# marl/l3embedding

Hardware: AMD Instinct MI355X
Metric: AVC training pairs/sec (1s audio + 224x224 frame) (higher is better)
Workload: dtype f32; 1 GPU; full cnn_L3_melspec2 AVC training step (audio+vision+fusion, fwd+bwd+Adam), batch 64 per GPU, global batch 64, fp32, inputs resident in HBM; global_batch=64, parallelism=dp1, fp32_conv=f4x4

## Files before the change

### l3embedding_amd/csrc/bn_fused.hip

```cpp
#include "kernels.h"
#include "device_common.h"

namespace l3 {



__device__ __forceinline__ void store_quad(void* base, int64_t q, f32x4 v, int obf) {
    if (obf) {
        bf16x4 h;
        h[0] = (__bf16)v.x; h[1] = (__bf16)v.y; h[2] = (__bf16)v.z; h[3] = (__bf16)v.w;
        __builtin_nontemporal_store(h, reinterpret_cast<bf16x4*>(base) + q);
    } else {
        __builtin_nontemporal_store(v, reinterpret_cast<f32x4*>(base) + q);
    }
}

template <bool XBF>
__device__ __forceinline__ f32x4 load_quad(const void* base, int64_t q) {
    if constexpr (XBF) {
        const u32x2 r = __builtin_nontemporal_load(reinterpret_cast<const u32x2*>(base) + q);
        return f32x4{__uint_as_float(r.x << 16), __uint_as_float(r.x & 0xffff0000u), __uint_as_float(r.y << 16),
                     __uint_as_float(r.y & 0xffff0000u)};
    } else {
        return __builtin_nontemporal_load(reinterpret_cast<const f32x4*>(base) + q);
// ... 545 lines not shown
    using ReduceFn = void (*)(const void*, const void*, const f32x4*, const f32x4*, const f32x4*, const f32x4*, float*, int64_t,
                              Pool2Geom, float, int);
    static const ReduceFn reduce_fns[8] = {
        bn_bwd_reduce_fast_kernel<false, false, false>, bn_bwd_reduce_fast_kernel<false, false, true>,
        bn_bwd_reduce_fast_kernel<false, true, false>,  bn_bwd_reduce_fast_kernel<false, true, true>,
        bn_bwd_reduce_fast_kernel<true, false, false>,  bn_bwd_reduce_fast_kernel<true, false, true>,
        bn_bwd_reduce_fast_kernel<true, true, false>,   bn_bwd_reduce_fast_kernel<true, true, true>};
    if (ready_part != nullptr) {
        launch_fast_final(BwdFinal{gamma, mean, var, dgamma, dbeta, cA, cB, cC, 1.0 / (double)rows, eps, training}, ready_part,
                          ready_blocks, C, s);
    } else {
        hipLaunchKernelGGL(reduce_fns[variant], dim3(nb_r), dim3(FB), 0, s, xv, dyv, sc4, sh4, reinterpret_cast<const f32x4*>(mean),
                           reinterpret_cast<const f32x4*>(var), part, n4, g, eps, relu);
        launch_fast_final(BwdFinal{gamma, mean, var, dgamma, dbeta, cA, cB, cC, 1.0 / (double)rows, eps, training}, part,
                          nb_r, C, s);
    }
    if (dx == nullptr) return;
    const int64_t work_a = pooled ? (int64_t)N * g.Hc * g.Wc * (C / 4) : n4;
    const int nb_a = fast_blocks(work_a);
    float* part2 = dbias ? part : nullptr;
    using ApplyFn = void (*)(const void*, const void*, const f32x4*, const f32x4*, const f32x4*, const f32x4*, const f32x4*, void*,
                             float*, int64_t, Pool2Geom, int, int);
    static const ApplyFn apply_fns[8] = {
        bn_bwd_apply_fast_kernel<false, false, false>, bn_bwd_apply_fast_kernel<false, false, true>,
        bn_bwd_apply_fast_kernel<false, true, false>,  bn_bwd_apply_fast_kernel<false, true, true>,
        bn_bwd_apply_fast_kernel<true, false, false>,  bn_bwd_apply_fast_kernel<true, false, true>,
        bn_bwd_apply_fast_kernel<true, true, false>,   bn_bwd_apply_fast_kernel<true, true, true>};
    hipLaunchKernelGGL(apply_fns[variant], dim3(nb_a), dim3(FB), 0, s, xv, dyv, sc4, sh4, reinterpret_cast<const f32x4*>(cA),
                       reinterpret_cast<const f32x4*>(cB), reinterpret_cast<const f32x4*>(cC), (void*)dx, part2, n4, g, relu,
                       dx_bf16);
    if (dbias) launch_fast_final(SumFinal{dbias}, part, nb_a, C, s);
}

}
```

### l3embedding_amd/csrc/elementwise.hip

```cpp
#include "kernels.h"

namespace l3 {

static constexpr int RED_BLOCK = 256;
static constexpr int RED_MAX_BLOCKS = 1024;
static constexpr int SMALLC_MAX = 16;

static inline int red_blocks(int64_t rows, int C) {
    int rows_per_pass = (C % 4 == 0 && C >= 4 && C <= 1024) ? (RED_BLOCK / (C / 4) > 0 ? RED_BLOCK / (C / 4) : 1) : RED_BLOCK;
    int64_t b = (rows + (int64_t)rows_per_pass * 16 - 1) / ((int64_t)rows_per_pass * 16);
    if (b < 1) b = 1;
    if (b > RED_MAX_BLOCKS) b = RED_MAX_BLOCKS;
    return (int)b;
}

size_t colreduce_scratch_floats(int64_t rows, int C) {
    const size_t a = (size_t)red_blocks(rows, C) * 2 * (size_t)(C < 4 ? 4 : C) + 64;
    const size_t b = bn_fast_ok(C) ? bn_fast_scratch_floats(C) : 0;
    return a > b ? a : b;
}

template <class F>
__global__ __launch_bounds__(RED_BLOCK) void colreduce_vec_kernel(F f, float* part, int64_t rows, int C) {
    __shared__ float sm[2][RED_BLOCK * 4];
// ... 494 lines not shown
    float best[4];
    int arg[4];
    gp_scan(x + (size_t)n * P * C + cb * 64 + cq * 4, P, C, pg, best, arg);
    gp_merge(sb, sa, pg, cq, best, arg);
    if (threadIdx.x < 64) y[(size_t)n * out_batch_stride + cb * 64 + threadIdx.x] = sb[0][threadIdx.x];
}
__global__ __launch_bounds__(256) void global_maxpool_bwd_kernel(const float* __restrict__ x, const float* __restrict__ dy,
                                                                 float* __restrict__ dx, int P, int C,
                                                                 int64_t out_batch_stride) {
    __shared__ float sb[16][64];
    __shared__ int sa[16][64];
    const int cb = blockIdx.x % (C / 64), n = blockIdx.x / (C / 64);
    const int cq = threadIdx.x & 15, pg = threadIdx.x >> 4;
    float best[4];
    int arg[4];
    const size_t base = (size_t)n * P * C + cb * 64 + cq * 4;
    gp_scan(x + base, P, C, pg, best, arg);
    gp_merge(sb, sa, pg, cq, best, arg);
    const gp4 d = *reinterpret_cast<const gp4*>(dy + (size_t)n * out_batch_stride + cb * 64 + cq * 4);
    int am[4];
#pragma unroll
    for (int e = 0; e < 4; ++e) am[e] = sa[0][cq * 4 + e];
    for (int p = pg; p < P; p += 16) {
        gp4 o;
#pragma unroll
        for (int e = 0; e < 4; ++e) o[e] = p == am[e] ? d[e] : 0.f;
        *reinterpret_cast<gp4*>(dx + base + (size_t)p * C) = o;
    }
}
static bool is_global_pool(const PoolGeom& g) {
    return g.Ho == 1 && g.Wo == 1 && g.padT == 0 && g.padL == 0 && g.ph == g.H && g.pw == g.W && g.C % 64 == 0 &&
           g.out_batch_stride % 4 == 0;
}

void maxpool_fwd(const float* x, float* y, const PoolGeom& g, hipStream_t s) {
    if (is_global_pool(g)) {
        hipLaunchKernelGGL(global_maxpool_fwd_kernel, dim3(g.N * (g.C / 64)), dim3(256), 0, s, x, y, g.H * g.W, g.C,
                           (int64_t)g.out_batch_stride);
        return;
    }
    const int64_t total = (int64_t)g.N * g.Ho * g.Wo * g.C;
    hipLaunchKernelGGL(maxpool_fwd_kernel, dim3(ew_blocks(total)), dim3(256), 0, s, x, y, g);
}
__global__ __launch_bounds__(256) void maxpool_bwd_kernel(const float* x, const float* dy, float* dx, PoolGeom g) {
    const int64_t total = (int64_t)g.N * g.Ho * g.Wo * g.C;
    for (int64_t i = (int64_t)blockIdx.x * 256 + threadIdx.x; i < total; i += (int64_t)gridDim.x * 256) {
        const int c = (int)(i % g.C);
        int64_t r = i / g.C;
        const int wo = (int)(r % g.Wo);
        r /= g.Wo;
        const int ho = (int)(r % g.Ho);
        const int n = (int)(r / g.Ho);
        const int h0 = ho * g.sh - g.padT, w0 = wo * g.sw - g.padL;
        float best = -INFINITY;
        int ba = -1, bb = -1;
        for (int a = 0; a < g.ph; ++a) {
            const int h = h0 + a;
            if ((unsigned)h >= (unsigned)g.H) continue;
            for (int b = 0; b < g.pw; ++b) {
                const int w = w0 + b;
                if ((unsigned)w >= (unsigned)g.W) continue;
                const float v = x[((size_t)(n * g.H + h) * g.W + w) * g.C + c];
                if (ba < 0 || v > best) { best = v; ba = a; bb = b; }
            }
        }
        const float d = dy[(size_t)n * g.out_batch_stride + ((size_t)ho * g.Wo + wo) * g.C + c];
// ... 32 lines not shown
        xa[i] = c == C ? 1.f : (x[r * C + c] - mean[c]) * (1.f / sqrtf(var[c] + eps));
    }
}
void bn_xhat_ones(const float* x, const float* mean, const float* var, float eps, float* xa, int64_t rows, int C,
                  hipStream_t s) {
    hipLaunchKernelGGL(bn_xhat_ones_kernel, dim3(ew_blocks(rows * (C + 1))), dim3(256), 0, s, x, mean, var, eps, xa, rows, C);
}

__global__ __launch_bounds__(256) void first_conv_grads_kernel(const float* __restrict__ gaug, const float* __restrict__ w,
                                                               const float* __restrict__ gamma, const float* __restrict__ beta,
                                                               float* __restrict__ dw, float* __restrict__ dgamma,
                                                               float* __restrict__ dbeta, float* __restrict__ dbias, int taps,
                                                               int C, int Co) {
    __shared__ double red[2][256];
    const int t = threadIdx.x;
    const int C1 = C + 1;
    for (int i = t; i < taps * C * Co; i += 256) {
        const int co = i % Co, ci = (i / Co) % C, tap = i / (Co * C);
        dw[i] = gamma[ci] * gaug[(tap * C1 + ci) * Co + co] + beta[ci] * gaug[(tap * C1 + C) * Co + co];
    }
    if (dbias != nullptr)
        for (int co = t; co < Co; co += 256) dbias[co] = gaug[((taps / 2) * C1 + C) * Co + co];
    for (int ci = 0; ci < C; ++ci) {
        double sg = 0.0, sb = 0.0;
        for (int i = t; i < taps * Co; i += 256) {
            const int co = i % Co, tap = i / Co;
            const double wv = (double)w[(tap * C + ci) * Co + co];
            sg += wv * (double)gaug[(tap * C1 + ci) * Co + co];
            sb += wv * (double)gaug[(tap * C1 + C) * Co + co];
        }
        red[0][t] = sg;
        red[1][t] = sb;
        __syncthreads();
        if (t == 0) {
            double a = 0.0, b = 0.0;
            for (int k = 0; k < 256; ++k) {
                a += red[0][k];
                b += red[1][k];
            }
            dgamma[ci] = (float)a;
            dbeta[ci] = (float)b;
        }
        __syncthreads();
    }
}
void first_conv_grads(const float* gaug, const float* w, const float* gamma, const float* beta, float* dw, float* dgamma,
                      float* dbeta, float* dbias, int taps, int C, int Co, hipStream_t s) {
    hipLaunchKernelGGL(first_conv_grads_kernel, dim3(1), dim3(256), 0, s, gaug, w, gamma, beta, dw, dgamma, dbeta, dbias, taps,
                       C, Co);
}

__global__ __launch_bounds__(256) void preprocess_video_kernel(const uint8_t* u8, float* out, int64_t n) {
    for (int64_t i = (int64_t)blockIdx.x * 256 + threadIdx.x; i < n; i += (int64_t)gridDim.x * 256) {
        const float f = (float)((double)u8[i] / 255.0);
        out[i] = 2.f * f - 1.f;
    }
}
__global__ __launch_bounds__(256) void preprocess_audio_kernel(const int16_t* pcm, float* out, int64_t n) {
    for (int64_t i = (int64_t)blockIdx.x * 256 + threadIdx.x; i < n; i += (int64_t)gridDim.x * 256)
        out[i] = (float)pcm[i] / 32768.f;
}
__global__ void labels_onehot_kernel(const int32_t* lab, float* out, int64_t n) {
    for (int64_t i = (int64_t)blockIdx.x * blockDim.x + threadIdx.x; i < n; i += (int64_t)gridDim.x * blockDim.x)
        out[i] = (float)lab[i];
}
void preprocess_video(const uint8_t* u8, float* out, int64_t n, hipStream_t s) {
    hipLaunchKernelGGL(preprocess_video_kernel, dim3(ew_blocks(n)), dim3(256), 0, s, u8, out, n);
}
void preprocess_audio(const int16_t* pcm, float* out, int64_t n, hipStream_t s) {
    hipLaunchKernelGGL(preprocess_audio_kernel, dim3(ew_blocks(n)), dim3(256), 0, s, pcm, out, n);
}
void labels_onehot(const int32_t* lab, float* out, int64_t n, hipStream_t s) {
    hipLaunchKernelGGL(labels_onehot_kernel, dim3(ew_blocks(n)), dim3(256), 0, s, lab, out, n);
}
// ... 231 lines not shown
```

### l3embedding_amd/csrc/engine.hip

```cpp
#include <hip/hip_runtime.h>
#include "knobs.h"

#include <cmath>
#include <cstdio>
#include <cstdlib>
#include <cstring>
#include <map>
#include <string>
#include <vector>

#include "../../include/l3hip.h"
#include "comm.h"
#include "kernels.h"

namespace {

using namespace l3;

static thread_local std::string g_create_error;

constexpr float BN_EPS = 1e-3f;
constexpr float BN_MOMENTUM = 0.99f;
constexpr float L2_WEIGHT = 1e-5f;
constexpr float ADAM_B1 = 0.9f, ADAM_B2 = 0.999f, ADAM_EPS = 1e-8f;
// ... 16 lines not shown

struct Param {
    std::string name;
    int ndim = 0;
    int64_t shape[4] = {1, 1, 1, 1};
    bool trainable = false;
    int kind = 0;
    int64_t numel = 0;
    int bucket = 0;
    float* d = nullptr;
    float* g = nullptr;
};

enum ConvFwd { CF_BF16_STORED, CF_BF16_CAST, CF_FIRST, CF_FP32 };
enum ConvWgrad { WG_AUG, WG_AUG_DEFERRED, WG_BF16_STORED, WG_BF16_CAST, WG_FP32 };
enum ConvDgrad { DG_NONE, DG_SMALL, DG_BF16_STORED, DG_BF16_CAST, DG_WINO, DG_FLIPPED };
struct ConvPlan {
    ConvFwd fwd = CF_FP32;
    bool wino_filter = false;
    int stat_mode = 0;
    ConvWgrad wgrad = WG_FP32;
    bool colsum = false;
    ConvDgrad dgrad = DG_NONE;
    int bwd_bn = -1;
    double fwd_executed = -1.0, fwd_bytes = 0.0, wg_executed = -1.0, wg_bytes = 0.0, dg_executed = -1.0, dg_bytes = 0.0;
};
enum BnStats { BS_PARTIALS, BS_FAST, BS_PLAIN, BS_MOVING };
enum BnBwd { BB_BY_FIRST_CONV, BB_FAST_POOLED, BB_FAST, BB_FAST_DEFERRED, BB_PLAIN };
struct BnPlan {
    BnStats stats = BS_MOVING;
    int stat_blocks = 0;
    BnBwd bwd = BB_PLAIN;
    int bwd_blocks = 0;
    double fwd_bytes = 0.0, bwd_bytes = 0.0;
};

struct Op {
    OpKind kind;
    std::string name;
    int in = 0, out = 0;
    int block = 0, bucket = 0;
    int kh = 0, kw = 0, cout = 0;
    bool same = false;
    ConvGeom geom{};
    ConvGeom dgeom{};
    int p_kernel = -1, p_bias = -1;
    float* wflip = nullptr;
    float *wino_uf = nullptr, *wino_ud = nullptr;
    int in_bn = -1;
    bool fused_first = false;
    bool defer_apply = false;
    int bn_defer = -1;
    float *xaug = nullptr, *gaug = nullptr;
    ConvGeom ageom{};
    int bn_follow = -1;
    bool need_dx = true;
    int dy_to_bn = -1;
    float* xwin = nullptr;
    int p_gamma = -1, p_beta = -1, p_mmean = -1, p_mvar = -1;
    bool fused_relu = false;
    bool prerelu = false;
    int fuse_pool = -1;
    int bias_param = -1;
    bool fused_into_bn = false;
    bool bias_by_bn = false;
    float *mean = nullptr, *var = nullptr, *scale = nullptr, *shift = nullptr;
    float *biased_mean = nullptr, *biased_var = nullptr;
    PoolGeom pg{};
    ConvPlan cp{};
    BnPlan bp{};
};

struct Tower {
    std::string prefix;
    std::vector<Tensor> t;
    std::vector<Op> ops;
    int nblocks = 0;
    int emb_conv_op = -1;
    bool training = false;
};

struct FrontendDef {
    int n_dft, n_hop, same, n_mels, sqrt_out, db, loglambda;
    const char* layer_name;
};

struct ProfRec {
    int family;
    hipEvent_t a, b;
    double flops;
    double executed;
// ... 889 lines not shown
                    const size_t sf = (size_t)conv_wino_stat_blocks_max(op.geom) * 2 * op.geom.Cout;
                    if (sf > stat_max) stat_max = sf;
                    const size_t sb = (size_t)conv_bf16_stat_blocks(op.geom) * 2 * op.geom.Cout;
                    if (e->cfg.dtype == L3_DTYPE_BF16 && sb > stat_max) stat_max = sb;
                    const size_t s1 = (size_t)conv_first_stat_blocks(op.geom) * 2 * op.geom.Cout;
                    if (s1 > stat_max) stat_max = s1;
                    const size_t sd = op.dy_to_bn >= 0 ? (size_t)conv_wino_stat_blocks_max(op.dgeom) * 2 * op.dgeom.Cout : 0;
                    if (sd > stat_max) stat_max = sd;
                    const size_t sdb = op.dy_to_bn >= 0 && e->cfg.dtype == L3_DTYPE_BF16
                                           ? (size_t)conv_bf16_stat_blocks(op.dgeom) * 2 * op.dgeom.Cout : 0;
                    if (sdb > stat_max) stat_max = sdb;
                }
                if (op.need_dx && conv_wino_floats(op.dgeom) &&
                    (rc = dev_alloc_t(e, &op.wino_ud, conv_wino_floats(op.dgeom))))
                    return rc;
                const size_t w = conv_wgrad_scratch_floats(op.geom);
                if (w > wg_max) wg_max = w;
                if (op.in_bn >= 0) {
                    if ((rc = dev_alloc_t(e, &op.xaug, (size_t)x.rows() * op.ageom.Cin))) return rc;
                    if ((rc = dev_alloc_t(e, &op.gaug, (size_t)op.kh * op.kw * op.ageom.Cin * op.cout))) return rc;
                    const size_t wa = conv_wgrad_scratch_floats(op.ageom);
                    if (wa > wg_max) wg_max = wa;
                }
                const size_t r = colreduce_scratch_floats(y.rows(), y.C);
                if (r > red_max) red_max = r;
            } else if (op.kind == OP_BN) {
                const int C = x.C;
                for (float** p : {&op.mean, &op.var, &op.scale, &op.shift, &op.biased_mean, &op.biased_var}) {
                    if ((rc = dev_alloc_t(e, p, (size_t)(C + 3) / 4 * 4))) return rc;
                    HIPCHK(e, hipMemset(*p, 0, (size_t)(C + 3) / 4 * 4 * 4));
                }
                const size_t r = colreduce_scratch_floats(x.rows(), C);
                if (r > red_max) red_max = r;
            }
        }
    }
    if (e->vis.ops.back().kind != OP_POOL || e->aud.ops.back().kind != OP_POOL) {
        e->err = "tower must end in a pooling layer";
        return L3_EINVAL;
    }
    if ((rc = dev_alloc_t(e, &e->red_scratch, red_max))) return rc;
    if ((rc = dev_alloc_t(e, &e->wg_scratch, wg_max))) return rc;
    if ((rc = dev_alloc_t(e, &e->sq_scratch, 2048))) return rc;
    if (stat_max && (rc = dev_alloc_t(e, &e->stat_scratch, stat_max))) return rc;
    {
        bool any_w4 = false;
        for (Tower* tw : {&e->vis, &e->aud})
            for (auto& op : tw->ops)
                if (op.kind == OP_CONV && (op.wino_uf || op.wino_ud)) any_w4 = true;
        if (any_w4 && e->cfg.dtype != L3_DTYPE_BF16 && (rc = dev_alloc_t(e, &e->w4_tail, conv_wino4_tail_scratch_bytes() / sizeof(float)))) return rc;
    }
    if (e->side) {
        if ((rc = dev_alloc_t(e, &e->red_scratch2, red_max))) return rc;
        if ((rc = dev_alloc_t(e, &e->wg_scratch2, wg_max))) return rc;
        if (stat_max && (rc = dev_alloc_t(e, &e->stat_scratch2, stat_max))) return rc;
    }
    return L3_OK;
}

int run_frontend(l3_engine* e) {
    int rc = rebuild_consts(e);
    if (rc) return rc;
    const FrontendCfg& f = e->fcfg;
    const int B = e->B;
    const int M = B * f.n_frames;
    if (f.factored) {
// ... 96 lines not shown
            p.wg_bytes = (double)x.rows() * op.ageom.Cin * 4.0 + (fb ? act_bytes(tw.t[fb->in]) + grad_bytes(tw.t[fb->out]) : grad_bytes(y));
            continue;
        }
        const bool wbf = bf16 && conv_wgrad_bf16_ok(op.geom);
        p.wgrad = !wbf ? WG_FP32 : x.d_bf16 && y.g_bf16 ? WG_BF16_STORED : WG_BF16_CAST;
        p.wg_executed = conv_wgrad_executed_flops(op.geom, wbf);
        p.wg_bytes = act_bytes(x) + grad_bytes(y) + wbytes;
        p.colsum = !op.bias_by_bn;
        if (!op.need_dx) continue;
        const bool dbf = bf16 && conv_bf16_ok(op.dgeom);
        p.dgrad = conv_dgrad_small_ok(op.geom) ? DG_SMALL
                  : dbf                        ? (y.g_bf16 ? DG_BF16_STORED : DG_BF16_CAST)
                  : op.wino_ud                 ? DG_WINO : DG_FLIPPED;
        p.dg_executed = op.wino_ud && !dbf ? conv_wino_executed_flops(op.dgeom) : -1.0;
        p.dg_bytes = grad_bytes(y) + grad_bytes(x) + wbytes;
        Op* bn = training && op.dy_to_bn >= 0 && e->stat_max > 0 ? &tw.ops[op.dy_to_bn] : nullptr;
        if (bn != nullptr && bn->fuse_pool >= 0 && (bn->xwin == nullptr || x.batch_stride != (int64_t)x.H * x.W * x.C)) bn = nullptr;
        if (bn == nullptr) continue;
        const bool bx = tw.t[bn->in].d_bf16;
        int blocks = -1;
        if (p.dgrad == DG_BF16_STORED && x.g_bf16 && bx && conv_bf16_halo_ok(op.dgeom)) blocks = conv_bf16_stat_blocks(op.dgeom);
        if (p.dgrad == DG_WINO && !x.g_bf16 && !bx && conv_wino_ok(op.dgeom)) blocks = conv_wino_stat_blocks(op.dgeom);
        if (blocks < 0) continue;
        if (!fits(op, blocks, op.dgeom.Cout)) return L3_ESTATE;
        p.bwd_bn = op.dy_to_bn;
        bn->bp.bwd_blocks = blocks;
    }
    for (auto& op : tw.ops) {
        if (op.kind != OP_BN) continue;
        const Tensor &x = tw.t[op.in], &y = tw.t[op.out];
        const Tensor& out = op.fuse_pool >= 0 ? tw.t[tw.ops[op.fuse_pool].out] : y;
        BnPlan& p = op.bp;
        p.stats = !training ? BS_MOVING : p.stat_blocks > 0 ? BS_PARTIALS : op.prerelu || x.d_bf16 ? BS_FAST : BS_PLAIN;
        p.bwd = training && op.fused_first ? BB_BY_FIRST_CONV : !bn_fast_ok(x.C) ? BB_PLAIN : op.fuse_pool >= 0 ? BB_FAST_POOLED
                : defers(op) ? BB_FAST_DEFERRED : BB_FAST;
        p.fwd_bytes = (!training ? 0.0 : p.stat_blocks > 0 ? (double)p.stat_blocks * 2 * x.C * 4 : act_bytes(x)) + act_bytes(x) + act_bytes(out);
        if (p.bwd == BB_BY_FIRST_CONV) p.fwd_bytes += act_bytes(x) + (double)x.rows() * (&op + 1)->ageom.Cin * 4.0;
        if (op.fuse_pool >= 0 && training && op.xwin != nullptr) p.fwd_bytes += (double)out.numel() * (x.d_bf16 ? 2.0 : 4.0);
        p.bwd_bytes = p.bwd == BB_PLAIN ? 2.0 * (act_bytes(x) + grad_bytes(y)) + grad_bytes(x)
                                        : (p.bwd_blocks > 0 ? (double)p.bwd_blocks * 2 * x.C * 4 : act_bytes(x) + grad_bytes(out)) +
                                              (p.bwd == BB_FAST_DEFERRED ? 0.0 : act_bytes(x) + grad_bytes(out) + grad_bytes(x));
    }
    return L3_OK;
}

void tower_forward(l3_engine* e, Tower& tw) {
    const bool training = tw.training;
    for (auto& op : tw.ops) {
        Tensor& x = tw.t[op.in];
        Tensor& y = tw.t[op.out];
        switch (op.kind) {
            case OP_CONV: {
                const ConvPlan& p = op.cp;
                const float *w = e->params[op.p_kernel].d, *bias = e->params[op.p_bias].d;
                float* part = p.stat_mode ? e->stat_scratch : nullptr;
                ProfScope ps(e, F_CONV_FWD, conv_flops(op.geom), op.name.c_str(), p.fwd_executed);
                ps.bytes(p.fwd_bytes);
                if (p.wino_filter) conv_wino_transform_weights(w, op.wino_uf, op.geom, false, e->stream);
                switch (p.fwd) {
                    case CF_BF16_STORED:
                        conv_weights_bf16(w, op.wflip, op.kh, op.kw, x.C, op.cout, true, e->stream);
                        conv_bf16_fwd(x.d, op.wflip, bias, y.d, op.geom, e->stream, true, part, p.stat_mode, y.d_bf16);
                        break;
                    case CF_BF16_CAST:
                        conv_flip_weights(w, op.wflip, op.kh, op.kw, x.C, op.cout, e->stream);
                        conv_bf16_fwd(x.d, op.wflip, bias, y.d, op.geom, e->stream);
                        break;
                    case CF_FIRST:
                        conv_first_fwd(x.d, w, bias, y.d, op.geom, e->stream, part, p.stat_mode, y.d_bf16);
                        break;
                    case CF_FP32:
                        conv_fwd(x.d, w, bias, y.d, op.geom, e->stream, p.wino_filter ? op.wino_uf : nullptr, part, p.stat_mode);
                        break;
                }
                break;
            }
            case OP_BN: {
                const BnPlan& p = op.bp;
                ProfScope ps(e, F_ELEMWISE, 0.0);
                ps.bytes(p.fwd_bytes);
                const float* gamma = e->params[op.p_gamma].d;
                const float* beta = e->params[op.p_beta].d;
                switch (p.stats) {
                    case BS_PARTIALS:
                        bn_stats_from_partials(e->stat_scratch, p.stat_blocks, e->params[op.bias_param].d, gamma, beta, op.mean, op.var,
                                               op.scale, op.shift, x.rows(), x.C, BN_EPS, op.prerelu ? 1 : 0, e->stream);
                        break;
                    case BS_FAST:
                        bn_stats_fast(x.d, gamma, beta, op.mean, op.var, op.scale, op.shift, e->red_scratch, x.rows(), x.C, BN_EPS,
                                      op.prerelu ? 1 : 0, e->stream, x.d_bf16 ? 1 : 0);
                        break;
                    case BS_PLAIN:
                        bn_stats(x.d, gamma, beta, op.mean, op.var, op.scale, op.shift, e->red_scratch, x.rows(), x.C, BN_EPS, e->stream);
                        break;
                    case BS_MOVING:
                        bn_scale_shift(gamma, beta, e->params[op.p_mmean].d, e->params[op.p_mvar].d, op.scale, op.shift, x.C, BN_EPS,
                                       e->stream);
                        break;
                }
                if (p.bwd == BB_BY_FIRST_CONV) bn_xhat_ones(x.d, op.mean, op.var, BN_EPS, (&op + 1)->xaug, x.rows(), x.C, e->stream);
                if (op.fuse_pool >= 0) {
                    Tensor& pl = tw.t[tw.ops[op.fuse_pool].out];
                    bn_relu_pool2_fwd(x.d, op.scale, op.shift, pl.d, x.N, x.H, x.W, x.C, pl.H, pl.W, pl.batch_stride,
                                      op.prerelu ? 2 : (op.fused_relu ? 1 : 0), e->stream, pl.d_bf16 ? 1 : 0, x.d_bf16 ? 1 : 0,
                                      training ? (void*)op.xwin : nullptr);
                } else if (y.d_bf16 || x.d_bf16) {
                    bn_apply_fast(x.d, op.scale, op.shift, y.d, x.rows(), x.C, op.fused_relu ? 1 : 0, e->stream, y.d_bf16 ? 1 : 0,
                                  x.d_bf16 ? 1 : 0);
                } else {
                    bn_apply(x.d, op.scale, op.shift, y.d, x.rows(), x.C, op.fused_relu ? 1 : 0, e->stream);
                }
                break;
            }
            case OP_RELU: {
                if (op.fused_into_bn) break;
                ProfScope ps(e, F_ELEMWISE, 0.0);
                ps.bytes(act_bytes(x) + act_bytes(y));
                relu_fwd(x.d, y.d, x.numel(), e->stream);
                break;
            }
            case OP_POOL: {
                if (op.fused_into_bn) break;
                ProfScope ps(e, F_ELEMWISE, 0.0);
                ps.bytes(act_bytes(x) + act_bytes(y));
                maxpool_fwd(x.d, y.d, op.pg, e->stream);
                break;
            }
            default: break;
        }
    }
}

BnBwdFuse bn_bwd_fuse(const Tower& tw, const Op& bn) {
    return BnBwdFuse{bn.fuse_pool >= 0 ? bn.xwin : tw.t[bn.in].d, bn.scale, bn.shift, bn.mean, bn.var, BN_EPS, bn.fused_relu ? 1 : 0};
}

void tower_backward_block(l3_engine* e, Tower& tw, int block) {
    const bool training = tw.training;
    for (int oi = (int)tw.ops.size() - 1; oi >= 0; --oi) {
        Op& op = tw.ops[oi];
        if (op.block != block) continue;
        Tensor& x = tw.t[op.in];
        Tensor& y = tw.t[op.out];
        switch (op.kind) {
            case OP_POOL: {
                if (op.fused_into_bn) break;
                ProfScope ps(e, F_ELEMWISE, 0.0);
                ps.bytes(act_bytes(x) + grad_bytes(y) + grad_bytes(x));
                maxpool_bwd(x.d, y.g, x.g, op.pg, e->stream);
                break;
            }
            case OP_RELU: {
                if (op.fused_into_bn) break;
                ProfScope ps(e, F_ELEMWISE, 0.0);
                ps.bytes(act_bytes(y) + grad_bytes(y) + grad_bytes(x));
                relu_bwd(y.d, y.g, x.g, x.numel(), e->stream);
                break;
            }
            case OP_BN: {
                const BnPlan& p = op.bp;
                if (p.bwd == BB_BY_FIRST_CONV) break;
                ProfScope ps(e, F_ELEMWISE, 0.0);
                ps.bytes(p.bwd_bytes);
                const float* mean = training ? op.mean : e->params[op.p_mmean].d;
                const float* var = training ? op.var : e->params[op.p_mvar].d;
                const float* gamma = e->params[op.p_gamma].d;
                float *dgamma = e->params[op.p_gamma].g, *dbeta = e->params[op.p_beta].g;
                if (p.bwd == BB_PLAIN) {
                    bn_bwd(x.d, y.d, y.g, gamma, mean, var, x.g, dgamma, dbeta, e->red_scratch, x.rows(), x.C, BN_EPS, op.fused_relu ? 1 : 0,
                           training ? 1 : 0, e->stream);
                    break;
                }
                const bool pooled = p.bwd == BB_FAST_POOLED, defer = p.bwd == BB_FAST_DEFERRED;
                const Tensor& dy = pooled ? tw.t[tw.ops[op.fuse_pool].out] : y;
                bn_bwd_fast(x.d, op.scale, op.shift, mean, var, gamma, dy.g, pooled ? 1 : 0, x.N, x.H, x.W, x.C, dy.H, dy.W,
                            pooled ? dy.batch_stride : (int64_t)x.H * x.W * x.C, defer ? nullptr : x.g, dgamma, dbeta,
                            defer ? nullptr : op.bias_param >= 0 ? e->params[op.bias_param].g : nullptr, e->red_scratch, BN_EPS,
                            pooled ? (op.prerelu ? 2 : 1) : (op.fused_relu ? 1 : 0), training ? 1 : 0, e->stream, x.g_bf16 ? 1 : 0,
                            x.d_bf16 ? 1 : 0, dy.g_bf16 ? 1 : 0, p.bwd_blocks > 0 ? e->stat_scratch : nullptr, p.bwd_blocks);
                break;
            }
            case OP_CONV: {
                const ConvPlan& p = op.cp;
                const float* w = e->params[op.p_kernel].d;
                if (p.wgrad == WG_AUG || p.wgrad == WG_AUG_DEFERRED) {
                    ProfScope ps(e, F_CONV_WGRAD, conv_flops(op.geom), op.name.c_str());
                    ps.bytes(p.wg_bytes);
                    const Op& bn = tw.ops[op.in_bn];
                    if (p.wgrad == WG_AUG_DEFERRED) {
                        const Op& fb = tw.ops[op.bn_defer];
                        const Tensor &bi = tw.t[fb.in], &bo = tw.t[fb.out];
                        const float* co = bn_bwd_fast_coeffs(e->red_scratch, op.cout);
                        const FirstWgFuse f{bi.d, bo.g, fb.scale, fb.shift, co, co + op.cout, co + 2 * op.cout, fb.fused_relu ? 1 : 0,
                                            bi.d_bf16 ? 1 : 0};
                        conv_wgrad(op.xaug, nullptr, op.gaug, e->wg_scratch, op.ageom, e->stream, false, false, &f);
                    } else {
                        conv_wgrad(op.xaug, y.g, op.gaug, e->wg_scratch, op.ageom, e->stream);
                    }
                    first_conv_grads(op.gaug, w, e->params[bn.p_gamma].d, e->params[bn.p_beta].d, e->params[op.p_kernel].g,
                                     e->params[bn.p_gamma].g, e->params[bn.p_beta].g,
// ... 1309 lines not shown
int l3_activation_numel(l3_engine* e, const char* name, int64_t* numel) {
    if (!e || !name || !numel) return L3_EINVAL;
    const std::string nm(name);
    if (nm == "h0") { *numel = (int64_t)e->B * (e->nv + e->na); return L3_OK; }
    if (nm == "h1") { *numel = (int64_t)e->B * e->head; return L3_OK; }
    if (nm == "logits" || nm == "probs") { *numel = (int64_t)e->B * 2; return L3_OK; }
    Tensor* t = nullptr;
    if (!find_tower_tensor(e, nm, &t)) {
        e->err = "unknown activation: " + nm;
        return L3_EINVAL;
    }
    *numel = t->numel();
    return L3_OK;
}

int l3_get_activation(l3_engine* e, const char* name, float* dst, int64_t numel) {
    int64_t n = 0;
    int rc = l3_activation_numel(e, name, &n);
    if (rc) return rc;
    if (n != numel) {
        e->err = "activation size mismatch";
        return L3_EINVAL;
    }
    HIPCHK(e, hipSetDevice(e->cfg.device));
    HIPCHK(e, l3::stream_wait(e->stream));
    const std::string nm(name);
    const float* src = nullptr;
    if (nm == "h0") src = e->h0;
    else if (nm == "h1") src = e->h1;
    else if (nm == "logits") src = e->logits;
    else if (nm == "probs") src = e->probs;
    else {
        Tensor* t = nullptr;
        find_tower_tensor(e, nm, &t);
        if (t->alias || t->d == nullptr) {
            e->err = "activation is not materialised (aliased into h0 or fused away)";
            return L3_EINVAL;
        }
        src = t->d;
        if (t->d_bf16) {
            std::vector<uint16_t> h((size_t)numel);
            HIPCHK(e, hipMemcpy(h.data(), src, (size_t)numel * 2, hipMemcpyDeviceToHost));
            l3::widen_bf16(dst, h.data(), (size_t)numel);
            return L3_OK;
        }
    }
    HIPCHK(e, hipMemcpy(dst, src, (size_t)numel * 4, hipMemcpyDeviceToHost));
    return L3_OK;
}

int l3_sync(l3_engine* e) {
    if (!e) return L3_EINVAL;
    HIPCHK(e, hipSetDevice(e->cfg.device));
    HIPCHK(e, l3::stream_wait(e->stream));
    if (e->side) HIPCHK(e, l3::stream_wait(e->side));
    prof_collect(e);
    return L3_OK;
}

int l3_set_tower_overlap(l3_engine* e, int on) {
    if (!e) return L3_EINVAL;
    HIPCHK(e, l3::stream_wait(e->stream));
    if (e->side) HIPCHK(e, l3::stream_wait(e->side));
    e->overlap = on != 0;
    return L3_OK;
}

int l3_profile_enable(l3_engine* e, int on) {
// ... 44 lines not shown
```

### l3embedding_amd/csrc/kernels.h

```cpp
#pragma once
#include <hip/hip_runtime.h>
#include <stdint.h>

#include <string>
#include <vector>

#include "host_common.h"

namespace l3 {

struct ConvGeom {
    int N, H, W, Cin;
    int Ho, Wo, Cout;
    int KH, KW, padT, padL;
    int f2x2 = 0;
    int solo = 0;
    int dynamic = 0;
    float* tail_scratch = nullptr;
    size_t tail_scratch_bytes = 0;
};
size_t conv_wino4_tail_scratch_bytes();

struct BnBwdFuse {
    const float* x;
// ... 79 lines not shown
                      int zero_debias, int step, hipStream_t s);
int* persistent_work_counters(hipStream_t s);

struct BnMovingEntry {
    float* moving;
    float* biased;
    const float* batch;
    int C;
    int off;
};
void bn_moving_update_all(const BnMovingEntry* tab_dev, int entries, int max_c, float momentum, int zero_debias, int64_t step,
                          hipStream_t s, const float* gathered = nullptr, int replicas = 1, int64_t stride = 0);
void bn_moving_pack(const BnMovingEntry* tab_dev, int entries, int max_c, float* packed, hipStream_t s);

bool bn_fast_ok(int C);
size_t bn_fast_scratch_floats(int C);
void bn_stats_fast(const float* x, const float* gamma, const float* beta, float* mean, float* var, float* scale,
                   float* shift, float* scratch, int64_t rows, int C, float eps, int prerelu, hipStream_t s, int x_bf16 = 0);
void bn_stats_from_partials(const float* part, int nblk, const float* pivot, const float* gamma, const float* beta,
                            float* mean, float* var, float* scale, float* shift, int64_t rows, int C, float eps,
                            int prerelu, hipStream_t s);
void bn_apply_fast(const float* x, const float* scale, const float* shift, float* y, int64_t rows, int C, int relu,
                   hipStream_t s, int out_bf16 = 0, int x_bf16 = 0);
void bn_relu_pool2_fwd(const float* x, const float* scale, const float* shift, float* p, int N, int H, int W, int C,
                       int Ho, int Wo, int64_t out_batch_stride, int mode, hipStream_t s, int out_bf16 = 0, int x_bf16 = 0,
                       void* xwin = nullptr);
void bn_bwd_fast(const float* x, const float* scale, const float* shift, const float* mean, const float* var,
                 const float* gamma, const float* dy, int pooled, int N, int H, int W, int C, int Ho, int Wo,
                 int64_t dy_batch_stride, float* dx, float* dgamma, float* dbeta, float* dbias, float* scratch,
                 float eps, int relu, int training, hipStream_t s, int dx_bf16 = 0, int x_bf16 = 0, int dy_bf16 = 0,
                 const float* ready_part = nullptr, int ready_blocks = 0);
const float* bn_bwd_fast_coeffs(const float* scratch, int C);

void relu_fwd(const float* x, float* y, int64_t n, hipStream_t s);
void relu_bwd(const float* y, const float* dy, float* dx, int64_t n, hipStream_t s);

struct PoolGeom {
    int N, H, W, C, Ho, Wo, ph, pw, sh, sw, padT, padL;
    int64_t out_batch_stride;
};
void maxpool_fwd(const float* x, float* y, const PoolGeom& g, hipStream_t s);
void maxpool_bwd(const float* x, const float* dy, float* dx, const PoolGeom& g, hipStream_t s);

void preprocess_video(const uint8_t* u8, float* out, int64_t n, hipStream_t s);
void preprocess_audio(const int16_t* pcm, float* out, int64_t n, hipStream_t s);
void labels_onehot(const int32_t* lab, float* out, int64_t n, hipStream_t s);

struct AugmentParams {
    int32_t start_x, start_y, flip, sat_first;
    float saturation, brightness;
};
constexpr int AUG_CROP = 224;
void augment_video(const uint8_t* u8, int N, int H, int W, const AugmentParams* params, uint8_t* out_u8, float* out_f32,
                   hipStream_t s);
void augment_audio(const int16_t* pcm, int N, int T, const double* u, int16_t* out_i16, float* out_f32, double* gains,
                   hipStream_t s);

struct FrontendCfg {
    int n_dft, n_hop, pad_left, n_frames, n_freq, n_mels;
    int sqrt_out;
    int db;
    int loglambda;
    int ncols_pad;
    int folded, ke, ko, nc;
    int factored, N1, N2;
};
void dft_pack_frames(const float* audio, const float* win, float* a1, int B, int T, const FrontendCfg& c, hipStream_t s);
void dft_twiddle(const float* y, const float* tw, float* a2, float* nyq, int frames, const FrontendCfg& c, hipStream_t s);
void frame_audio_folded(const float* audio, float* fe, float* fo, int B, int T, const FrontendCfg& c, hipStream_t s);
void frame_audio(const float* audio, float* frames, int B, int T, const FrontendCfg& c, hipStream_t s);
void dft_fused(const float* audio, const float* win, const float* b1, const float* b2, const float* tw, const float* melw,
               const int* mel_start, const int* mel_len, const int* mel_off, float* out, int B, int T, const FrontendCfg& c,
               hipStream_t s);
// ... 71 lines not shown
```

Before: 2017 pairs/s.

## Fuse tower-final BN+ReLU with global max-pool in forward and backward

When a tower's last BN (with fused ReLU) feeds a global max-pool, the forward now computes BN+ReLU on the fly and reduces straight to the pooled output plus argmax indices, so the full post-BN activation is never written. The backward rebuilds the sparse pooled gradient from the stored indices inside the BN backward reduce and apply kernels, skipping the separate maxpool backward pass and its dense gradient tensor. It also swaps the serial 256-element double reduction in first_conv_grads for a tree reduction. In exchange it adds scratch and index buffers, and the BN output tensor is no longer readable for debugging.

```diff
diff --git a/l3embedding_amd/csrc/bn_fused.hip b/l3embedding_amd/csrc/bn_fused.hip
--- a/l3embedding_amd/csrc/bn_fused.hip
+++ b/l3embedding_amd/csrc/bn_fused.hip
@@ -601,4 +601,172 @@
     if (dbias) launch_fast_final(SumFinal{dbias}, part, nb_a, C, s);
 }
 
-}
+constexpr int GP_MAX_SLICES = 32;
+static inline int gpool_slices(int P) {
+    const int s = (P + 15) / 16;
+    return s < 1 ? 1 : s > GP_MAX_SLICES ? GP_MAX_SLICES : s;
+}
+size_t bn_relu_gpool_scratch_floats(int N, int C) { return (size_t)N * GP_MAX_SLICES * C * 2; }
+
+__global__ __launch_bounds__(FB) void bn_relu_gpool_fwd_kernel(const f32x4* __restrict__ x, const f32x4* scale, const f32x4* shift,
+                                                              float* __restrict__ pval, int* __restrict__ pidx, int P, int C4,
+                                                              int slices, int chunk) {
+    __shared__ f32x4 sb[FB];
+    __shared__ int sa[FB][4];
+    const int t = threadIdx.x, c4 = t % C4, pg = t / C4, G = FB / C4;
+    const int n = blockIdx.x / slices, sl = blockIdx.x - n * slices;
+    const int p0 = sl * chunk, p1 = min(P, p0 + chunk);
+    const f32x4 sc = scale[c4], sh = shift[c4];
+    const f32x4* xb = x + (size_t)n * P * C4 + c4;
+    f32x4 best = {-INFINITY, -INFINITY, -INFINITY, -INFINITY};
+    int arg[4] = {0x7fffffff, 0x7fffffff, 0x7fffffff, 0x7fffffff};
+#pragma unroll 4
+    for (int p = p0 + pg; p < p1; p += G) {
+        const f32x4 v = relu4(bn_pre(xb[(size_t)p * C4], sc, sh));
+#pragma unroll
+        for (int e = 0; e < 4; ++e)
+            if (v[e] > best[e] || arg[e] == 0x7fffffff) {
+                best[e] = v[e];
+                arg[e] = p;
+            }
+    }
+    sb[t] = best;
+#pragma unroll
+    for (int e = 0; e < 4; ++e) sa[t][e] = arg[e];
+    __syncthreads();
+    if (pg == 0) {
+        for (int k = 1; k < G; ++k) {
+            const f32x4 vb = sb[k * C4 + c4];
+#pragma unroll
+            for (int e = 0; e < 4; ++e) {
+                const int va = sa[k * C4 + c4][e];
+                if (vb[e] > best[e] || (vb[e] == best[e] && va < arg[e])) {
+                    best[e] = vb[e];
+                    arg[e] = va;
+                }
+            }
+        }
+        const size_t o = ((size_t)blockIdx.x * C4 + c4) * 4;
+        *reinterpret_cast<f32x4*>(pval + o) = best;
+#pragma unroll
+        for (int e = 0; e < 4; ++e) pidx[o + e] = arg[e];
+    }
+}
+__global__ __launch_bounds__(256) void bn_relu_gpool_merge_kernel(const float* __restrict__ pval, const int* __restrict__ pidx,
+                                                                  float* __restrict__ p, int* __restrict__ win, int N, int C,
+                                                                  int slices, int64_t out_batch_stride) {
+    const int i = blockIdx.x * 256 + threadIdx.x;
+    if (i >= N * C) return;
+    const int n = i / C, c = i - n * C;
+    float vs[GP_MAX_SLICES];
+    int as[GP_MAX_SLICES];
+#pragma unroll
+    for (int sl = 0; sl < GP_MAX_SLICES; ++sl) {
+        const size_t o = ((size_t)n * slices + (sl < slices ? sl : 0)) * C + c;
+        vs[sl] = pval[o];
+        as[sl] = sl < slices ? pidx[o] : 0x7fffffff;
+    }
+    float b = -INFINITY;
+    int a = 0x7fffffff;
+#pragma unroll
+    for (int sl = 0; sl < GP_MAX_SLICES; ++sl)
+        if (as[sl] != 0x7fffffff && (vs[sl] > b || a == 0x7fffffff)) {
+            b = vs[sl];
+            a = as[sl];
+        }
+    p[(size_t)n * out_batch_stride + c] = b;
+    win[i] = a;
+}
+void bn_relu_gpool_fwd(const float* x, const float* scale, const float* shift, float* p, int* win, float* scratch, int N, int P, int C,
+                       int64_t out_batch_stride, hipStream_t s) {
+    const int slices = gpool_slices(P), chunk = (P + slices - 1) / slices;
+    float* pval = scratch;
+    int* pidx = reinterpret_cast<int*>(scratch + (size_t)N * slices * C);
+    hipLaunchKernelGGL(bn_relu_gpool_fwd_kernel, dim3(N * slices), dim3(FB), 0, s, reinterpret_cast<const f32x4*>(x),
+                       reinterpret_cast<const f32x4*>(scale), reinterpret_cast<const f32x4*>(shift), pval, pidx, P, C / 4, slices, chunk);
+    hipLaunchKernelGGL(bn_relu_gpool_merge_kernel, dim3((N * C + 255) / 256), dim3(256), 0, s, pval, pidx, p, win, N, C, slices,
+                       out_batch_stride);
+}
+
+__global__ __launch_bounds__(256) void bn_gpool_bwd_reduce_kernel(BwdFinal fin, const float* __restrict__ x, const float* scale,
+                                                                  const float* shift, const float* __restrict__ dp,
+                                                                  const int* __restrict__ win, int N, int P, int C,
+                                                                  int64_t dp_batch_stride) {
+    const int lane = threadIdx.x & 63, c = blockIdx.x * 4 + (threadIdx.x >> 6);
+    if (c >= C) return;
+    const float sc = scale[c], sh = shift[c], mu = fin.mean[c], rs = rsqrtf(fin.var[c] + fin.eps);
+    double s0 = 0.0, s1 = 0.0;
+    for (int n = lane; n < N; n += 64) {
+        const int w = win[(size_t)n * C + c];
+        const float xv = x[((size_t)n * P + w) * C + c];
+        const float d = fmaf(xv, sc, sh) > 0.f ? dp[(size_t)n * dp_batch_stride + c] : 0.f;
+        s0 += (double)d;
+        s1 += (double)(d * ((xv - mu) * rs));
+    }
+#pragma unroll
+    for (int off = 32; off > 0; off >>= 1) {
+        s0 += __shfl_xor(s0, off, 64);
+        s1 += __shfl_xor(s1, off, 64);
+    }
+    if (lane == 0) fin(c, s0, s1);
+}
+__global__ __launch_bounds__(FB) void bn_gpool_bwd_apply_kernel(const f32x4* __restrict__ x, const float* __restrict__ dp,
+                                                               const int* __restrict__ win, const f32x4* scale, const f32x4* shift,
+                                                               const f32x4* cA, const f32x4* cB, const f32x4* cC,
+                                                               f32x4* __restrict__ dx, float* part, int64_t n4, int C4, int c4_shift,
+                                                               int P, int64_t dp_batch_stride) {
+    constexpr int U = 4;
+    const int c4 = (int)threadIdx.x % C4;
+    const f32x4 sc = scale[c4], sh = shift[c4], A = cA[c4], B = cB[c4], Cc = cC[c4];
+    f32x4 a0 = {0.f, 0.f, 0.f, 0.f};
+    const int64_t stride = (int64_t)gridDim.x * (FB * U);
+    for (int64_t q = (int64_t)blockIdx.x * (FB * U) + threadIdx.x; q < n4; q += stride) {
+        f32x4 v[U], g[U];
+        int w[U][4], pp[U];
+#pragma unroll
+        for (int u = 0; u < U; ++u)
+            if (q + u * FB < n4) {
+                v[u] = x[q + u * FB];
+                const int row = (int)((q + u * FB) >> c4_shift), n = row / P;
+                pp[u] = row - n * P;
+                g[u] = *reinterpret_cast<const f32x4*>(dp + (size_t)n * dp_batch_stride + c4 * 4);
+                const int4 wi = *reinterpret_cast<const int4*>(win + ((size_t)n * C4 + c4) * 4);
+                w[u][0] = wi.x; w[u][1] = wi.y; w[u][2] = wi.z; w[u][3] = wi.w;
+            }
+#pragma unroll
+        for (int u = 0; u < U; ++u)
+            if (q + u * FB < n4) {
+                const f32x4 pre = bn_pre(v[u], sc, sh);
+                f32x4 d;
+#pragma unroll
+                for (int e = 0; e < 4; ++e) d[e] = pp[u] == w[u][e] && pre[e] > 0.f ? g[u][e] : 0.f;
+                const f32x4 o = A * d + (B * v[u] + Cc);
+                dx[q + u * FB] = o;
+                a0 += o;
+            }
+    }
+    if (part != nullptr) block_write_partials(a0, a0, part, C4);
+}
+void bn_gpool_bwd(const float* x, const float* scale, const float* shift, const float* mean, const float* var, const float* gamma,
+                  const float* dp, const int* win, int N, int P, int C, int64_t dp_batch_stride, float* dx, float* dgamma,
+                  float* dbeta, float* dbias, float* scratch, float eps, int training, hipStream_t s) {
+    const int64_t rows = (int64_t)N * P, n4 = rows * (C / 4);
+    float* part = scratch;
+    float* cA = scratch + (size_t)FAST_MAX_BLOCKS * 2 * C;
+    float* cB = cA + C;
+    float* cC = cB + C;
+    hipLaunchKernelGGL(bn_gpool_bwd_reduce_kernel, dim3((C + 3) / 4), dim3(256), 0, s,
+                       BwdFinal{gamma, mean, var, dgamma, dbeta, cA, cB, cC, 1.0 / (double)rows, eps, training}, x, scale, shift, dp, win,
+                       N, P, C, dp_batch_stride);
+    int64_t nb = (n4 + FB * 4 - 1) / (FB * 4);
+    if (nb > FAST_MAX_BLOCKS) nb = FAST_MAX_BLOCKS;
+    int c4_shift = 0;
+    while ((1 << c4_shift) < C / 4) ++c4_shift;
+    hipLaunchKernelGGL(bn_gpool_bwd_apply_kernel, dim3((int)nb), dim3(FB), 0, s, reinterpret_cast<const f32x4*>(x), dp, win,
+                       reinterpret_cast<const f32x4*>(scale), reinterpret_cast<const f32x4*>(shift), reinterpret_cast<const f32x4*>(cA),
+                       reinterpret_cast<const f32x4*>(cB), reinterpret_cast<const f32x4*>(cC), reinterpret_cast<f32x4*>(dx),
+                       dbias ? part : nullptr, n4, C / 4, c4_shift, P, dp_batch_stride);
+    if (dbias) launch_fast_final(SumFinal{dbias}, part, (int)nb, C, s);
+}
+
+}
diff --git a/l3embedding_amd/csrc/elementwise.hip b/l3embedding_amd/csrc/elementwise.hip
--- a/l3embedding_amd/csrc/elementwise.hip
+++ b/l3embedding_amd/csrc/elementwise.hip
@@ -550,6 +550,7 @@
     return g.Ho == 1 && g.Wo == 1 && g.padT == 0 && g.padL == 0 && g.ph == g.H && g.pw == g.W && g.C % 64 == 0 &&
            g.out_batch_stride % 4 == 0;
 }
+bool maxpool_is_global(const PoolGeom& g) { return is_global_pool(g); }
 
 void maxpool_fwd(const float* x, float* y, const PoolGeom& g, hipStream_t s) {
     if (is_global_pool(g)) {
@@ -648,14 +649,16 @@
         red[0][t] = sg;
         red[1][t] = sb;
         __syncthreads();
+        for (int h = 128; h > 0; h >>= 1) {
+            if (t < h) {
+                red[0][t] += red[0][t + h];
+                red[1][t] += red[1][t + h];
+            }
+            __syncthreads();
+        }
         if (t == 0) {
-            double a = 0.0, b = 0.0;
-            for (int k = 0; k < 256; ++k) {
-                a += red[0][k];
-                b += red[1][k];
-            }
-            dgamma[ci] = (float)a;
-            dbeta[ci] = (float)b;
+            dgamma[ci] = (float)red[0][0];
+            dbeta[ci] = (float)red[1][0];
         }
         __syncthreads();
     }
diff --git a/l3embedding_amd/csrc/engine.hip b/l3embedding_amd/csrc/engine.hip
--- a/l3embedding_amd/csrc/engine.hip
+++ b/l3embedding_amd/csrc/engine.hip
@@ -72,6 +72,8 @@
     int stat_blocks = 0;
     BnBwd bwd = BB_PLAIN;
     int bwd_blocks = 0;
+    int end_pool = -1;
+    bool in_bn_end = false;
     double fwd_bytes = 0.0, bwd_bytes = 0.0;
 };
 
@@ -97,6 +99,8 @@
     bool need_dx = true;
     int dy_to_bn = -1;
     float* xwin = nullptr;
+    int* gwin = nullptr;
+    float* gscratch = nullptr;
     int p_gamma = -1, p_beta = -1, p_mmean = -1, p_mvar = -1;
     bool fused_relu = false;
     bool prerelu = false;
@@ -1052,6 +1056,11 @@
                 }
                 const size_t r = colreduce_scratch_floats(x.rows(), C);
                 if (r > red_max) red_max = r;
+                if (oi + 2 == tw.ops.size() && tw.ops[oi + 1].kind == OP_POOL && maxpool_is_global(tw.ops[oi + 1].pg) && bn_fast_ok(C) &&
+                    op.fused_relu && !op.prerelu && op.fuse_pool < 0 && !x.d_bf16 && !x.g_bf16) {
+                    if ((rc = dev_alloc_t(e, &op.gwin, (size_t)x.N * C))) return rc;
+                    if ((rc = dev_alloc_t(e, &op.gscratch, bn_relu_gpool_scratch_floats(x.N, C)))) return rc;
+                }
             }
         }
     }
@@ -1214,11 +1223,21 @@
         const Tensor& out = op.fuse_pool >= 0 ? tw.t[tw.ops[op.fuse_pool].out] : y;
         BnPlan& p = op.bp;
         p.stats = !training ? BS_MOVING : p.stat_blocks > 0 ? BS_PARTIALS : op.prerelu || x.d_bf16 ? BS_FAST : BS_PLAIN;
+        if (training && op.gwin != nullptr && maxpool_is_global((&op + 1)->pg) && knob_int("L3_TOWER_END_FUSE", 1)) {
+            p.end_pool = (int)(&op - tw.ops.data()) + 1;
+            tw.ops[p.end_pool].bp.in_bn_end = true;
+        }
         p.bwd = training && op.fused_first ? BB_BY_FIRST_CONV : !bn_fast_ok(x.C) ? BB_PLAIN : op.fuse_pool >= 0 ? BB_FAST_POOLED
                 : defers(op) ? BB_FAST_DEFERRED : BB_FAST;
         p.fwd_bytes = (!training ? 0.0 : p.stat_blocks > 0 ? (double)p.stat_blocks * 2 * x.C * 4 : act_bytes(x)) + act_bytes(x) + act_bytes(out);
         if (p.bwd == BB_BY_FIRST_CONV) p.fwd_bytes += act_bytes(x) + (double)x.rows() * (&op + 1)->ageom.Cin * 4.0;
         if (op.fuse_pool >= 0 && training && op.xwin != nullptr) p.fwd_bytes += (double)out.numel() * (x.d_bf16 ? 2.0 : 4.0);
+        if (p.end_pool >= 0) {
+            const Tensor& pl = tw.t[tw.ops[p.end_pool].out];
+            p.fwd_bytes = (p.stat_blocks > 0 ? (double)p.stat_blocks * 2 * x.C * 4 : act_bytes(x)) + act_bytes(x) + 3.0 * act_bytes(pl);
+            p.bwd_bytes = act_bytes(x) + grad_bytes(x) + 3.0 * grad_bytes(pl);
+            continue;
+        }
         p.bwd_bytes = p.bwd == BB_PLAIN ? 2.0 * (act_bytes(x) + grad_bytes(y)) + grad_bytes(x)
                                         : (p.bwd_blocks > 0 ? (double)p.bwd_blocks * 2 * x.C * 4 : act_bytes(x) + grad_bytes(out)) +
                                               (p.bwd == BB_FAST_DEFERRED ? 0.0 : act_bytes(x) + grad_bytes(out) + grad_bytes(x));
@@ -1281,7 +1300,10 @@
                         break;
                 }
                 if (p.bwd == BB_BY_FIRST_CONV) bn_xhat_ones(x.d, op.mean, op.var, BN_EPS, (&op + 1)->xaug, x.rows(), x.C, e->stream);
-                if (op.fuse_pool >= 0) {
+                if (p.end_pool >= 0) {
+                    const Tensor& pl = tw.t[tw.ops[p.end_pool].out];
+                    bn_relu_gpool_fwd(x.d, op.scale, op.shift, pl.d, op.gwin, op.gscratch, x.N, x.H * x.W, x.C, pl.batch_stride, e->stream);
+                } else if (op.fuse_pool >= 0) {
                     Tensor& pl = tw.t[tw.ops[op.fuse_pool].out];
                     bn_relu_pool2_fwd(x.d, op.scale, op.shift, pl.d, x.N, x.H, x.W, x.C, pl.H, pl.W, pl.batch_stride,
                                       op.prerelu ? 2 : (op.fused_relu ? 1 : 0), e->stream, pl.d_bf16 ? 1 : 0, x.d_bf16 ? 1 : 0,
@@ -1302,7 +1324,7 @@
                 break;
             }
             case OP_POOL: {
-                if (op.fused_into_bn) break;
+                if (op.fused_into_bn || op.bp.in_bn_end) break;
                 ProfScope ps(e, F_ELEMWISE, 0.0);
                 ps.bytes(act_bytes(x) + act_bytes(y));
                 maxpool_fwd(x.d, y.d, op.pg, e->stream);
@@ -1326,7 +1348,7 @@
         Tensor& y = tw.t[op.out];
         switch (op.kind) {
             case OP_POOL: {
-                if (op.fused_into_bn) break;
+                if (op.fused_into_bn || op.bp.in_bn_end) break;
                 ProfScope ps(e, F_ELEMWISE, 0.0);
                 ps.bytes(act_bytes(x) + grad_bytes(y) + grad_bytes(x));
                 maxpool_bwd(x.d, y.g, x.g, op.pg, e->stream);
@@ -1348,6 +1370,13 @@
                 const float* var = training ? op.var : e->params[op.p_mvar].d;
                 const float* gamma = e->params[op.p_gamma].d;
                 float *dgamma = e->params[op.p_gamma].g, *dbeta = e->params[op.p_beta].g;
+                if (p.end_pool >= 0) {
+                    const Tensor& pl = tw.t[tw.ops[p.end_pool].out];
+                    bn_gpool_bwd(x.d, op.scale, op.shift, mean, var, gamma, pl.g, op.gwin, x.N, x.H * x.W, x.C, pl.batch_stride, x.g, dgamma,
+                                 dbeta, op.bias_param >= 0 ? e->params[op.bias_param].g : nullptr, e->red_scratch, BN_EPS, training ? 1 : 0,
+                                 e->stream);
+                    break;
+                }
                 if (p.bwd == BB_PLAIN) {
                     bn_bwd(x.d, y.d, y.g, gamma, mean, var, x.g, dgamma, dbeta, e->red_scratch, x.rows(), x.C, BN_EPS, op.fused_relu ? 1 : 0,
                            training ? 1 : 0, e->stream);
@@ -2723,8 +2752,11 @@
     else if (nm == "probs") src = e->probs;
     else {
         Tensor* t = nullptr;
-        find_tower_tensor(e, nm, &t);
-        if (t->alias || t->d == nullptr) {
+        const Tower* tw = find_tower_tensor(e, nm, &t);
+        bool unwritten = false;
+        for (const auto& op : tw->ops)
+            if (op.kind == OP_BN && op.bp.end_pool >= 0 && &tw->t[op.out] == t) unwritten = true;
+        if (t->alias || t->d == nullptr || unwritten) {
             e->err = "activation is not materialised (aliased into h0 or fused away)";
             return L3_EINVAL;
         }
diff --git a/l3embedding_amd/csrc/kernels.h b/l3embedding_amd/csrc/kernels.h
--- a/l3embedding_amd/csrc/kernels.h
+++ b/l3embedding_amd/csrc/kernels.h
@@ -135,6 +135,13 @@
                  const float* ready_part = nullptr, int ready_blocks = 0);
 const float* bn_bwd_fast_coeffs(const float* scratch, int C);
 
+size_t bn_relu_gpool_scratch_floats(int N, int C);
+void bn_relu_gpool_fwd(const float* x, const float* scale, const float* shift, float* p, int* win, float* scratch, int N, int P, int C,
+                       int64_t out_batch_stride, hipStream_t s);
+void bn_gpool_bwd(const float* x, const float* scale, const float* shift, const float* mean, const float* var, const float* gamma,
+                  const float* dp, const int* win, int N, int P, int C, int64_t dp_batch_stride, float* dx, float* dgamma,
+                  float* dbeta, float* dbias, float* scratch, float eps, int training, hipStream_t s);
+
 void relu_fwd(const float* x, float* y, int64_t n, hipStream_t s);
 void relu_bwd(const float* y, const float* dy, float* dx, int64_t n, hipStream_t s);
 
@@ -142,6 +149,7 @@
     int N, H, W, C, Ho, Wo, ph, pw, sh, sw, padT, padL;
     int64_t out_batch_stride;
 };
+bool maxpool_is_global(const PoolGeom& g);
 void maxpool_fwd(const float* x, float* y, const PoolGeom& g, hipStream_t s);
 void maxpool_bwd(const float* x, const float* dy, float* dx, const PoolGeom& g, hipStream_t s);
 
```

Measured after the change: 2031 pairs/s (median of 6 runs). No clear change (+0.7%).
